# xmindflow/deformableLKA

Hardware: AMD Instinct MI355X
Metric: 3D D-LKA fwd+bwd volumes/sec (64x128x128, b2) (higher is better)
Workload: dtype f32; 1 GPU; 3D D-LKA Former Synapse 64x128x128 patch: fwd+bwd of its 21 D-LKA attention blocks (6x(32,32^3)+6x(64,16^3)+6x(128,8^3)+3x(256,4^3)) + grad all-reduce + SGD update; batch_per_gpu=2, global_batch=2, parallelism=dp1, block_params=15390693, hipgraph=True, weight_gradients_on_side_stream=True, allreduce_overlap=False, allreduce_split_block=0

## Files before the change

### deformablelka_amd/_lib.py

```python
from __future__ import annotations

import ctypes
import os
from ctypes import POINTER, c_char_p, c_int, c_int32, c_int64, c_size_t, c_void_p

import torch

_HERE = os.path.dirname(os.path.abspath(__file__))
LIB_PATH = os.path.join(_HERE, "_lib", "libdlka_hip.so")

DLKA_F32, DLKA_BF16, DLKA_F64 = 0, 1, 2
DLKA_TILES_MAX_T, DLKA_TILES_K_MAX = 64, 32
DLKA_TILES_IDENTITY, DLKA_TILES_SOFTMAX, DLKA_TILES_SIGMOID = 0, 1, 2
LKA3D_SYNAPSE, LKA3D_ACDC = 0, 1


class ConvGeom(ctypes.Structure):
    _fields_ = [(n, c_int32) for n in (
        "B", "C", "D", "H", "W", "Cout", "kd", "kh", "kw", "sd", "sh", "sw", "pd", "ph", "pw", "dd", "dh", "dw",
        "group", "deformable_group", "im2col_step")]


LKA3D_FIELDS = ("proj_1_w", "proj_1_b", "conv0_w", "conv0_b", "conv_spatial_w", "conv_spatial_b", "offset_w", "offset_b",
                "deform_w", "deform_b", "conv1_w", "conv1_b", "proj_2_w", "proj_2_b")
# ... 66 lines not shown
    "dlka_lka3d_tokens_supported": (c_int, [c_int] * 6),
    "dlka_lka3d_tokens_saved_bytes": (c_size_t, [c_int] * 6),
    "dlka_lka3d_tokens_workspace_bytes": (c_size_t, [c_int] * 6),
    "dlka_lka3d_attention_tokens_forward": (c_int, [c_void_p, POINTER(Lka3dPtrs), c_void_p, c_void_p, c_size_t, c_void_p, c_size_t]
                                            + [c_int] * 6 + [c_void_p]),
    "dlka_lka3d_attention_tokens_forward_prepared": (c_int, [c_void_p, POINTER(Lka3dPtrs), c_void_p, c_void_p, c_size_t, c_void_p, c_size_t]
                                                     + [c_int] * 6 + [c_void_p]),
    "dlka_lka3d_tokens_prepare_plan_bytes": (c_size_t, [c_int]),
    "dlka_lka3d_tokens_prepare_plan": (c_int, [c_int, POINTER(Lka3dPtrs), POINTER(c_void_p), POINTER(c_size_t), POINTER(c_int), c_int, c_void_p, c_size_t]),
    "dlka_lka3d_tokens_prepare_run": (c_int, [c_void_p, c_void_p, c_int, c_void_p]),
    "dlka_lka3d_tokens_prepare_run_range": (c_int, [c_void_p, c_void_p, c_int, c_int, c_int, c_void_p]),
    "dlka_lka3d_tokens_partials_bytes_v": (c_size_t, [c_int] * 7),
    "dlka_wgrad_finalize_plan_bytes": (c_size_t, [c_int]),
    "dlka_wgrad_finalize_plan_init": (c_int, [c_void_p, c_size_t, c_int]),
    "dlka_lka3d_attention_tokens_backward_deferred_v": (c_int, [c_void_p, POINTER(Lka3dPtrs), c_void_p, c_void_p, c_size_t, c_void_p,
                                                               POINTER(Lka3dPtrs), c_void_p, c_size_t, c_void_p, c_size_t, c_void_p, c_int,
                                                               c_int, c_int, c_int, c_int, c_int, c_int, c_int, c_void_p]),
    "dlka_lka3d_attention_tokens_backward_phase_v": (c_int, [c_void_p, POINTER(Lka3dPtrs), c_void_p, c_void_p, c_size_t, c_void_p,
                                                            POINTER(Lka3dPtrs), c_void_p, c_size_t, c_void_p, c_size_t, c_void_p, c_int, c_int,
                                                            c_int, c_int, c_int, c_int, c_int, c_int, c_int, c_void_p]),
    "dlka_wgrad_finalize_plan_seal": (c_int, [c_void_p]),
    "dlka_wgrad_finalize_run_slot": (c_int, [c_void_p, c_int, c_void_p]),
    "dlka_wgrad_finalize_run": (c_int, [c_void_p, c_void_p, c_int, c_int, c_void_p]),
    "dlka_lka3d_attention_tokens_backward": (c_int, [c_void_p, POINTER(Lka3dPtrs), c_void_p, c_void_p, c_size_t, c_void_p,
                                                     POINTER(Lka3dPtrs), c_void_p, c_size_t] + [c_int] * 6 + [c_void_p]),
    "dlka_layernorm_tokens_forward": (c_int, [c_void_p, c_int] + [c_void_p] * 6 + [c_int] * 3 + [ctypes.c_float, c_int, c_void_p]),
    "dlka_layernorm_tokens_backward": (c_int, [c_void_p] * 9 + [c_int] * 4 + [c_void_p]),
    "dlka_scale_residual_forward": (c_int, [c_void_p] * 4 + [c_int64, c_int, c_int, c_void_p]),
    "dlka_scale_residual_backward": (c_int, [c_void_p] * 5 + [c_int64, c_int, c_int, c_void_p]),
    "dlka_batchnorm_cl_forward": (c_int, [c_void_p] * 5 + [c_int] + [c_void_p] * 2 + [c_int64, c_int, ctypes.c_float, ctypes.c_float, c_int, c_void_p]),
    "dlka_batchnorm_cl_backward": (c_int, [c_void_p] * 5 + [c_int] + [c_void_p] * 5 + [c_int64, c_int, ctypes.c_float, c_int, c_void_p]),
    "dlka_channel_scale": (c_int, [c_void_p] * 3 + [c_int, c_int64, c_int, c_int, c_void_p]),
    "dlka_batchnorm_planar_forward": (c_int, [c_void_p] * 6 + [c_int, c_int, c_int64, ctypes.c_float, c_void_p]),
    "dlka_batchnorm_planar_backward": (c_int, [c_void_p] * 8 + [c_int, c_int, c_int64, c_void_p]),
    "dlka_pointwise_planar_forward": (c_int, [c_void_p] * 4 + [c_int, c_int, c_int, c_int64, c_void_p]),
    "dlka_pointwise_planar_backward": (c_int, [c_void_p] * 6 + [c_int, c_int, c_int, c_int64, c_void_p]),
    "dlka_tblock3d_supported": (c_int, [c_int] * 6),
    "dlka_tblock3d_saved_bytes": (c_size_t, [c_int] * 6),
    "dlka_tblock3d_workspace_bytes": (c_size_t, [c_int] * 6),
    "dlka_tblock3d_forward": (c_int, [c_void_p, c_int, POINTER(TBlock3dPtrs), POINTER(Lka3dPtrs), c_void_p, c_int, c_void_p, c_void_p, c_void_p, c_size_t,
                                      c_void_p, c_size_t] + [c_int] * 5 + [ctypes.c_float, ctypes.c_float, c_int, c_void_p]),
    "dlka_tblock3d_backward": (c_int, [POINTER(TBlock3dPtrs), POINTER(Lka3dPtrs), c_void_p, c_int, c_void_p, c_void_p, c_void_p, c_size_t, c_void_p,
                                       POINTER(TBlock3dPtrs), POINTER(Lka3dPtrs), c_void_p, c_size_t] + [c_int] * 6 + [c_void_p]),
    "dlka_deform_conv2d_sample_index_path": (c_int, [c_void_p] * 3 + [_G, c_int, c_int, c_void_p]),
    "dlka_deform_dwconv2d_cl_workspace": (c_size_t, [_G, c_int, c_int]),
    "dlka_deform_dwconv2d_forward_cl": (c_int, [c_void_p] * 5 + [c_size_t, _G, c_int, c_void_p]),
    "dlka_deform_dwconv2d_backward_cl": (c_int, [c_void_p] * 8 + [c_size_t, _G, c_int, c_void_p]),
    "dlka_lka3d_force_wgrad_gather": (c_int, [c_int]),
    "dlka_fork_stats": (c_int, [c_int, POINTER(ctypes.c_int64), POINTER(ctypes.c_int64)]),
    "dlka_env_refresh": (None, []),
    "dlka_dwconv_lds_launch_count": (ctypes.c_long, []),
    "dlka_conv_brick_launch_count": (ctypes.c_long, []),
    "dlka_dwpair_launch_count": (ctypes.c_long, []),
    "dlka_dwconv_2p_launch_count": (ctypes.c_long, []),
    "dlka_conv_kw_launch_count": (ctypes.c_long, []),
    "dlka_lka3d_tokens_supported_v": (c_int, [c_int] * 7),
    "dlka_lka3d_tokens_saved_bytes_v": (c_size_t, [c_int] * 7),
    "dlka_lka3d_tokens_workspace_bytes_v": (c_size_t, [c_int] * 7),
    "dlka_lka3d_attention_tokens_forward_v": (c_int, [c_void_p, POINTER(Lka3dPtrs), c_void_p, c_void_p, c_size_t, c_void_p, c_size_t]
                                              + [c_int] * 7 + [c_void_p]),
    "dlka_lka3d_attention_tokens_backward_v": (c_int, [c_void_p, POINTER(Lka3dPtrs), c_void_p, c_void_p, c_size_t, c_void_p,
                                                       POINTER(Lka3dPtrs), c_void_p, c_size_t] + [c_int] * 7 + [c_void_p]),
    "dlka_lka3d_tokens_saved_offsets_v": (c_int, [c_int] * 7 + [POINTER(c_size_t)]),
    "dlka_tblock3d_saved_offsets_v": (c_int, [c_int] * 7 + [POINTER(c_size_t)]),
    "dlka_tblock3d_saved_activations_v": (c_int, [c_int] * 7 + [POINTER(c_size_t)]),
    "dlka_tblock3d_supported_v": (c_int, [c_int] * 7),
    "dlka_tblock3d_saved_bytes_v": (c_size_t, [c_int] * 7),
    "dlka_tblock3d_workspace_bytes_v": (c_size_t, [c_int] * 7),
    "dlka_tblock3d_forward_v": (c_int, [c_void_p, c_int, POINTER(TBlock3dPtrs), POINTER(Lka3dPtrs), c_void_p, c_int, c_void_p, c_void_p, c_void_p, c_size_t,
                                        c_void_p, c_size_t] + [c_int] * 5 + [ctypes.c_float, ctypes.c_float, c_int, c_int, c_void_p]),
    "dlka_tblock3d_backward_v": (c_int, [POINTER(TBlock3dPtrs), POINTER(Lka3dPtrs), c_void_p, c_int, c_void_p, c_void_p, c_void_p, c_size_t, c_void_p,
                                         POINTER(TBlock3dPtrs), POINTER(Lka3dPtrs), c_void_p, c_size_t] + [c_int] * 7 + [c_void_p]),
    "dlka_tblock3d_backward_phase_v": (c_int, [POINTER(TBlock3dPtrs), POINTER(Lka3dPtrs), c_void_p, c_int, c_void_p, c_void_p, c_void_p, c_size_t, c_void_p,
                                         POINTER(TBlock3dPtrs), POINTER(Lka3dPtrs), c_void_p, c_size_t] + [c_int] * 8 + [c_void_p]),
    "dlka_tiles_gather": (c_int, [c_void_p] + [c_int] * 4 + [POINTER(c_int), c_int, POINTER(c_int)] + [c_int] * 7 + [ctypes.c_float, c_void_p, c_void_p]),
    "dlka_tiles_blend": (c_int, [c_void_p, c_int, c_int, c_int, ctypes.c_float] + [c_void_p] * 3 + [c_int] * 3
                         + [POINTER(c_int), c_int, POINTER(c_int)] + [c_int] * 4 + [c_void_p]),
    "dlka_tiles_finalize": (c_int, [c_void_p] * 2 + [c_int] * 10 + [c_void_p] * 3),
    "dlka_tiles_launch_count": (ctypes.c_long, []),
    "dlka_trace_start": (c_int, [c_int, c_void_p]),
    "dlka_trace_mark": (c_int, [c_void_p]),
    "dlka_trace_stop": (c_int, []),
    "dlka_trace_count": (c_int, []),
    "dlka_trace_get": (c_int, [c_int, ctypes.c_char_p, c_size_t, POINTER(ctypes.c_float)]),
}


def bind(cdll: ctypes.CDLL) -> ctypes.CDLL:
    for name, (res, args) in SIGNATURES.items():
        fn = getattr(cdll, name)
        fn.restype = res
        fn.argtypes = args
    if cdll.dlka_abi_version() != 1:
        raise RuntimeError("libdlka ABI version mismatch")
    return cdll


_lib = None
_test_backend = False


def get_lib() -> ctypes.CDLL:
    global _lib
    if _lib is None:
        if not os.path.exists(LIB_PATH):
            raise RuntimeError(
# ... 56 lines not shown
```

### deformablelka_amd/csrc/cl_host_ops.hip

```cpp
#include <atomic>
#include <mutex>

#include "cl_host.h"

namespace dlka {

int make_same_conv(const dlka_conv_geom *c, SameConv &s)
{
    if (!c) return DLKA_ERR_NULL;
    if (c->B <= 0 || c->C <= 0 || c->D <= 0 || c->H <= 0 || c->W <= 0 || c->Cout <= 0) return DLKA_ERR_SHAPE;
    if (c->kd <= 0 || c->kh <= 0 || c->kw <= 0 || c->dd <= 0 || c->dh <= 0 || c->dw <= 0) return DLKA_ERR_SHAPE;
    if (c->group <= 0 || c->C % c->group || c->Cout % c->group) return DLKA_ERR_GROUP;
    if (c->sd != 1 || c->sh != 1 || c->sw != 1) return DLKA_ERR_UNSUPPORTED;
    if (dlka_conv_out_size(c->D, c->pd, c->dd, c->kd, 1) != c->D || dlka_conv_out_size(c->H, c->ph, c->dh, c->kh, 1) != c->H ||
        dlka_conv_out_size(c->W, c->pw, c->dw, c->kw, 1) != c->W)
        return DLKA_ERR_UNSUPPORTED;
    const long N = (long)c->D * c->H * c->W;
    if (N > (1l << 30) || (long)c->B * N > (1l << 30)) return DLKA_ERR_SHAPE;
    s.B = c->B; s.D = c->D; s.H = c->H; s.W = c->W; s.N = (int)N; s.M = (int)(c->B * N);
    s.Cin = c->C; s.Cout = c->Cout; s.group = c->group;
    s.kd = c->kd; s.kh = c->kh; s.kw = c->kw; s.pd = c->pd; s.ph = c->ph; s.pw = c->pw;
    s.dd = c->dd; s.dh = c->dh; s.dw = c->dw; s.K = c->kd * c->kh * c->kw;
    s.act_bf16 = 0;
    return DLKA_OK;
// ... 293 lines not shown
}

size_t deform_scratch_floats(const SameConv &s)
{
    DeformBwdArgs a;
    fill_deform_bwd(a, s);
    return cl_deform_bwd2_scratch_floats(a);
}

static bool samp_f16(const SameConv &s)
{
    static const bool on = [] { const char *e = getenv("DLKA_SAMP_F16"); return !(e && e[0] == '0') && getenv("DLKA_EXACT_FP32") == nullptr; }();
    return on && !s.act_bf16;
}

int deform_backward(const SameConv &s, const float *x, const float *off, const float *w, const float *gout, float *gx, float *goff,
                    float *gw, float *gb, float *wp, float *part, float *scratch, hipStream_t st, FinalizeJob *defer, bool gx_zeroed,
                    bool goff_zeroed, int goff_cpad, float *samp, const float *wp16)
{
    if (gx || goff) {
        if (w) DLKA_TRY(launch_cl_prep_weight(w, wp, s.Cout, s.Cin, s.K, s.Cout, s.Cin, 2, st));
        DeformBwdArgs a;
        fill_deform_bwd(a, s);
        a.in = x; a.off = off; a.g = gout; a.wp = wp; a.gx = gx; a.goff = goff; a.gx_zeroed = gx_zeroed ? 1 : 0; a.goff_zeroed = goff_zeroed ? 1 : 0; a.goff_cpad = goff_cpad;
        a.samp = goff ? samp : nullptr;
        a.samp_f16 = (a.samp && samp_f16(s)) ? 1 : 0;
        a.wp16 = deform_b16() ? wp16 : nullptr;
        DLKA_TRY(launch_cl_deform_bwd2(a, scratch, st));
    }
    if (gw) {
        WgradArgs a;
        memset(&a, 0, sizeof(a));
        a.g = gout; a.in = x; a.off = off; a.part = part; a.samp = samp;
        a.samp_f16 = (samp && samp_f16(s)) ? 1 : 0;
        {
            static const bool b16 = [] { const char *e = getenv("DLKA_SAMP_B16MFMA"); return !(e && e[0] == '0'); }();
            a.samp_b16mfma = (a.samp_f16 && b16) ? 1 : 0;
        }
        copy_geom(a, s);
        a.Cin = s.Cin; a.Cout = s.Cout;
        a.act_bf16 = s.act_bf16;
        DLKA_TRY(launch_cl_wgrad<float>(1, 0, a, gw, gb, st, defer));
    } else if (gb) {
        if (s.act_bf16) return DLKA_ERR_UNSUPPORTED;
        DLKA_TRY(launch_cl_colsum(gout, gb, s.M, s.Cout, st));
    }
    return DLKA_OK;
}

int pointwise_pair(const SameConv &s, int bwd, const float *in, const float *wp1, const float *bias1, const float *wp2, const float *bias2,
                   const float *a, const float *b, float *out1, float *out1b, float *out2, hipStream_t st, const ZeroBatch *ride)
{
    const bool unfused = getenv("DLKA_PW_UNFUSED") != nullptr;
    if (unfused || s.Cin != 32 || s.Cin != s.Cout || s.K != 1) return DLKA_ERR_UNSUPPORTED;
    PwPairArgs pa;
    memset(&pa, 0, sizeof(pa));
    pa.in = in; pa.wp1 = wp1; pa.bias1 = bias1; pa.wp2 = wp2; pa.bias2 = bias2; pa.a = a; pa.b = b;
    pa.out1 = out1; pa.out1b = out1b; pa.out2 = out2; pa.M = s.M; pa.C = s.Cin; pa.bwd = bwd; pa.act_bf16 = s.act_bf16;
    if (ride) pa.zero = *ride;
    return launch_cl_pointwise_pair(pa, st);
}

static std::atomic<int> g_wgrad_gather{-1};
bool wgrad_gather()
{
    int v = g_wgrad_gather.load(std::memory_order_acquire);
    if (v < 0) {
        int want = getenv("DLKA_WGRAD_GATHER") != nullptr ? 1 : 0;
        if (g_wgrad_gather.compare_exchange_strong(v, want, std::memory_order_acq_rel)) v = want;
    }
    return v != 0;
}

void add_job(PrepBatch &pb, const void *src, float *dst, int Cout, int Cin, int K, int KP, int NP, int mode)
{
    PrepJob &j = pb.j[pb.njobs++];
    j.src = (const float *)src; j.dst = dst; j.Cout = Cout; j.Cin = Cin; j.K = K; j.KP = KP; j.NP = NP; j.mode = mode;
    if (!fork_env().prep_tiled && (mode & 7) <= 2) j.mode |= 32;
    j.n = (mode == 3 || mode == 4) ? (long)Cin * K : (long)K * KP * NP;
    pb.total += j.n;
}

}

using namespace dlka;

extern "C" {

void dlka_env_refresh(void)
{
    fork_env_load();
}

int dlka_lka3d_force_wgrad_gather(int on)
{
    const int old = wgrad_gather() ? 1 : 0;
    g_wgrad_gather.store(on ? 1 : 0, std::memory_order_release);
    return old;
}

}
```

### deformablelka_amd/csrc/cl_pointwise.hip

```cpp
#include "cl_args.h"
#include "dlka_kernels.h"

namespace dlka {

template <typename T, int KW = 1>
__global__ __launch_bounds__(64 * KW, 2) void cl_pointwise_kernel(IgemmArgs p)
{
    constexpr unsigned SB = sizeof(T);
    const T *auxp = reinterpret_cast<const T *>(p.aux), *aux2p = reinterpret_cast<const T *>(p.aux2);
    T *outp = reinterpret_cast<T *>(p.out), *out2p = reinterpret_cast<T *>(p.out2);
    const int lane = threadIdx.x & 63, kwave = KW > 1 ? (int)(threadIdx.x >> 6) : 0, i = lane & 31, h = lane >> 5;
    if (p.zero_xblocks && (int)blockIdx.x >= (int)gridDim.x - p.zero_xblocks) {
        if (kwave == 0) zero_batch_block(p.zero, (blockIdx.x - (gridDim.x - p.zero_xblocks)) * gridDim.y + blockIdx.y, lane, 64);
        return;
    }
    const int mbase = blockIdx.x * 32, n0 = blockIdx.y * 32;
    const int m = mbase + i, n = n0 + i;
    const BufRsrc rin = make_rsrc(p.in, (size_t)p.M * p.Cin * SB);
    const BufRsrc rw = make_rsrc(p.wp, (size_t)p.CinP * p.NP * 4);
    const unsigned abase = m < p.M ? (unsigned)m * (unsigned)p.Cin * SB + 16u * SB * h : DLKA_OOB;
    const unsigned bbase = ((unsigned)(16 * h) * (unsigned)p.NP + (unsigned)n) * 4u;
    const unsigned bstep = (unsigned)p.NP * 4u;
    f32x16 acc;
#pragma unroll
    for (int r = 0; r < 16; ++r) acc[r] = 0.f;
    float auxv[16], aux2v[16];
    const bool n_ok = n < p.Cout;
    constexpr bool B16 = sizeof(T) == 2;
    const bool odd = i & 1;
    unsigned auxw[8], aux2w[8];
    auto pair_request = [&](const T *src, int r) -> unsigned {
        const int mrow = mbase + (r & 3) + 8 * (r >> 2) + 4 * h + (odd ? 1 : 0);
        return (n_ok && mrow < p.M) ? *reinterpret_cast<const unsigned *>(src + ((long)mrow * p.Cout + (n & ~1))) : 0u;
    };
    auto pair_finish = [&](unsigned own, float &x0, float &x1) {
        const unsigned oth = lane_xor1(own);
        x0 = __uint_as_float(odd ? (oth & 0xffff0000u) : (own << 16));
        x1 = __uint_as_float(odd ? (own & 0xffff0000u) : (oth << 16));
    };
    if (p.epi >= 2 && kwave == 0) {
        if (B16) {
#pragma unroll
            for (int r = 0; r < 16; r += 2) {
                auxw[r >> 1] = pair_request(auxp, r);
                aux2w[r >> 1] = p.epi == 4 ? pair_request(aux2p, r) : 0u;
            }
        } else {
#pragma unroll
            for (int r = 0; r < 16; ++r) {
                const int mr = mbase + (r & 3) + 8 * (r >> 2) + 4 * h;
                const bool ok = n_ok && mr < p.M;
                auxv[r] = ok ? act_load1(auxp, (long)mr * p.Cout + n) : 0.f;
// ... 189 lines not shown
#pragma unroll
        for (int r = 0; r < 16; ++r) acc[r] = 0.f;
#pragma unroll
        for (int u = 0; u < NTC; ++u) {
            float b[16];
#pragma unroll
            for (int s = 0; s < 16; ++s) b[s] = buf_load_f32(rw1, (unsigned)((u * 32 + 16 * h + s) * C + n) * 4u);
#pragma unroll
            for (int s = 0; s < 16; ++s) acc = mfma_32x32x2(a[u][s >> 2][s & 3], b[s], acc);
        }
        const float bias = (!p.bwd && p.bias1) ? p.bias1[n] : 0.f;
        float t1[16], t2[16];
#pragma unroll
        for (int r = 0; r < 16; ++r) {
            const float t = acc[r] + bias;
            if (p.bwd) { t1[r] = t * av[r]; t2[r] = t * bv2[r]; }
            else { t1[r] = t; t2[r] = av[r] * t; }
        }
        store_tile(o1, nt, t1);
        store_tile(o1b, nt, t2);
#pragma unroll
        for (int r = 0; r < 16; ++r) Tm[((r & 3) + 8 * (r >> 2) + 4 * h) * LD + n] = stored(p.bwd ? t1[r] : t2[r]);
    }
    wave_sync();
    f32x4 a2[NTC][4];
#pragma unroll
    for (int u = 0; u < NTC; ++u)
#pragma unroll
        for (int e = 0; e < 4; ++e) a2[u][e] = *reinterpret_cast<const f32x4 *>(Tm + i * LD + u * 32 + 16 * h + 4 * e);
#pragma unroll 1
    for (int nt = 0; nt < NTC; ++nt) {
        const int n = nt * 32 + i;
        float res[16];
        if (!p.bwd) load_tile(bp, nt, res);
        f32x16 acc;
#pragma unroll
        for (int r = 0; r < 16; ++r) acc[r] = 0.f;
#pragma unroll
        for (int u = 0; u < NTC; ++u) {
            float b[16];
#pragma unroll
            for (int s = 0; s < 16; ++s) b[s] = buf_load_f32(rw2, (unsigned)((u * 32 + 16 * h + s) * C + n) * 4u);
#pragma unroll
            for (int s = 0; s < 16; ++s) acc = mfma_32x32x2(a2[u][s >> 2][s & 3], b[s], acc);
        }
        const float bias = (!p.bwd && p.bias2) ? p.bias2[n] : 0.f;
        float y[16];
#pragma unroll
        for (int r = 0; r < 16; ++r) y[r] = p.bwd ? acc[r] : acc[r] + bias + res[r];
        store_tile(o2, nt, y);
    }
}

int launch_cl_pointwise_pair(const PwPairArgs &a, hipStream_t st)
{
    if ((a.C != 32 && a.C != 64) || (long)a.M * a.C * 4 >= (1l << 31)) return DLKA_ERR_UNSUPPORTED;
    PwPairArgs ax = a;
    ax.zero_blocks = 0;
    unsigned blocks = (unsigned)cdiv(a.M, 32);
    if (a.zero.n > 0) {
        if (a.zero.overflow) return DLKA_ERR_WORKSPACE;
        unsigned blk = 0;
        for (int r = 0; r < a.zero.n; ++r) {
            if ((uintptr_t)a.zero.p[r] & 15) return DLKA_ERR_UNSUPPORTED;
            ax.zero.block0[r] = blk;
            blk += (unsigned)cdivl(a.zero.cnt[r], 4096);
        }
        ax.zero.block0[a.zero.n] = blk;
        ax.zero_blocks = (int)blk;
        blocks += blk;
    }
    dim3 grid(blocks), block(64);
    if (a.act_bf16) {
        if (a.C == 32) { auto k = cl_pointwise_pair_kernel<bf16_t, 1>; DLKA_LAUNCH(k, grid, block, 0, st, ax); }
        else { auto k = cl_pointwise_pair_kernel<bf16_t, 2>; DLKA_LAUNCH(k, grid, block, 0, st, ax); }
    } else {
        if (a.C == 32) { auto k = cl_pointwise_pair_kernel<float, 1>; DLKA_LAUNCH(k, grid, block, 0, st, ax); }
        else { auto k = cl_pointwise_pair_kernel<float, 2>; DLKA_LAUNCH(k, grid, block, 0, st, ax); }
    }
    DLKA_CHECK_LAUNCH();
    return DLKA_OK;
}

int launch_cl_pointwise(const IgemmArgs &a, hipStream_t st)
{
    if (a.K != 1 || a.split_bf16 || a.Cin % 32 || a.CinP != a.Cin || a.NP % 32) return DLKA_ERR_UNSUPPORTED;
    if ((long)a.M * a.Cin * 4 >= (1l << 31) || (long)a.CinP * a.NP * 4 >= (1l << 31)) return DLKA_ERR_UNSUPPORTED;
    dim3 grid(cdiv(a.M, 32), a.NP / 32), block(64);
    IgemmArgs ax = a;
    ax.zero_xblocks = 0;
    if (a.zero.n > 0) {
        if (a.zero.overflow) return DLKA_ERR_WORKSPACE;
        unsigned blk = 0;
        for (int r = 0; r < a.zero.n; ++r) {
            if ((uintptr_t)a.zero.p[r] & 15) return DLKA_ERR_UNSUPPORTED;
            ax.zero.block0[r] = blk;
            blk += (unsigned)cdivl(a.zero.cnt[r], 4096);
        }
        ax.zero.block0[a.zero.n] = blk;
        ax.zero_xblocks = (int)cdiv((int)blk, (int)grid.y);
        grid.x += ax.zero_xblocks;
    }
    const char *ekw = getenv("DLKA_PW_KW");
    const bool kw4 = ekw ? atoi(ekw) == 4 : ((long)cdiv(a.M, 32) * (a.NP / 32) <= 256 && a.CinP >= 128);
    if (kw4) {
        block = dim3(256);
        if (a.act_bf16) { auto k = cl_pointwise_kernel<bf16_t, 4>; DLKA_LAUNCH(k, grid, block, 0, st, ax); }
        else { auto k = cl_pointwise_kernel<float, 4>; DLKA_LAUNCH(k, grid, block, 0, st, ax); }
    } else if (a.act_bf16) { auto k = cl_pointwise_kernel<bf16_t>; DLKA_LAUNCH(k, grid, block, 0, st, ax); }
    else { auto k = cl_pointwise_kernel<float>; DLKA_LAUNCH(k, grid, block, 0, st, ax); }
    DLKA_CHECK_LAUNCH();
    return DLKA_OK;
}

}
```

### deformablelka_amd/csrc/dlka_kernels.h

```cpp
#pragma once
#include "cl_args.h"
#include "dlka_common.h"

namespace dlka {

int deform_pick_cob(int Og);
int deform_fwd_wt_floats(const Geom &g);
template <typename T>
int launch_relayout_weight(const T *w, float *wt, int group, int Og, int Cg, int K, int OgP, hipStream_t st);
template <typename T, int NOFF>
int launch_deform_fwd(const T *x, const T *off, const T *w, const T *bias, T *out, float *wt, const Geom &g, hipStream_t st);
template <typename T, int NOFF>
int launch_deform_bwd_input_offset(const T *x, const T *off, const float *wt, int OgP, const T *gout,
                                   float *gx32, T *goff, const Geom &g, hipStream_t st);
template <typename T, int NOFF>
int launch_deform_bwd_weight(const T *x, const T *off, const T *gout, float *gw32, const Geom &g, hipStream_t st);
template <typename T>
int launch_bias_grad(const T *gout, T *gb, int B, int Cout, int No, hipStream_t st);
template <typename T>
int launch_cast_from_f32(const float *src, T *dst, long n, hipStream_t st);
template <typename T>
int launch_sample_index(const T *off, int32_t *idx, uint8_t *mask, const Geom &g, int path, hipStream_t st);
template <typename T>
int launch_sample_index2(const T *off, int32_t *idx, uint8_t *mask, const Geom &g, int path, hipStream_t st);

template <int NOFF> int launch_deform_fwd_f64(const double *x, const double *off, const double *w, const double *bias, double *out, const Geom &g, hipStream_t st);
template <int NOFF> int launch_deform_bwd_f64(const double *x, const double *off, const double *w, const double *gout, double *gx, double *goff, double *gw, double *gb,
                                              const Geom &g, hipStream_t st);
int launch_conv_fwd_f64(const double *x, const double *w, const double *bias, double *out, const Geom &g, hipStream_t st);
int launch_conv_bwd_f64(const double *x, const double *w, const double *gout, double *gx, double *gw, double *gb, const Geom &g, hipStream_t st);

int conv_fwd_wt_floats(const Geom &g);
int conv_bwd_wb_floats(const Geom &g);
template <typename T>
int launch_conv_fwd(const T *x, const T *w, const T *bias, T *out, float *wt, const Geom &g, hipStream_t st);
template <typename T>
int launch_conv_bwd_data(const T *gout, const T *w, T *gx, float *wb, const Geom &g, hipStream_t st);
size_t conv_bwd_weight_part_floats(const Geom &g, size_t elem_bytes);
template <typename T>
int launch_conv_bwd_weight(const T *x, const T *gout, float *gw32, const Geom &g, hipStream_t st, float *part = nullptr);

int launch_zero(void *ptr, size_t bytes, hipStream_t st);
struct ZeroBatch;
int launch_zero_batch(ZeroBatch &b, hipStream_t st);
template <typename T> int launch_gelu_fwd(const T *x, T *y, long n, hipStream_t st);
template <typename T> int launch_gelu_bwd(const T *x, const T *gy, T *gx, long n, hipStream_t st);
template <typename T> int launch_mul_fwd(const T *a, const T *b, T *y, long n, hipStream_t st);
template <typename T> int launch_mul_bwd(const T *a, const T *b, const T *gy, T *ga, T *gb, long n, hipStream_t st);
template <typename T> int launch_add_fwd(const T *a, const T *b, T *y, long n, hipStream_t st);
template <typename T> int launch_gelu_bwd_sum(const T *x, const T *g1, const T *g2, T *gx, long n, hipStream_t st);

int launch_cl_prep_weight(const float *w, float *wp, int Cout, int Cin, int K, int KP, int NP, int mode, hipStream_t st);
int launch_cl_prep_batch(const PrepBatch &b, hipStream_t st);
int cl_prep_table_blocks(const PrepJob &j);
int launch_cl_prep_table(const PrepJob *jobs_dev, const int *first_dev, int job_lo, int job_hi, int nblocks, hipStream_t st);
int cl_igemm_pick_splits(int M, int units, int epi, int K);
int launch_cl_pointwise(const IgemmArgs &a, hipStream_t st);
int launch_cl_pointwise_pair(const PwPairArgs &a, hipStream_t st);
int launch_cl_conv_wave(int amode, int omode, const IgemmArgs &a, int splits, hipStream_t st);
bool cl_conv_kw_applies(int amode, int omode, int split_bf16, int K, int epi, int NP, bool act_bf16, bool volume);
int launch_cl_conv_kw(int amode, int omode, const IgemmArgs &a, hipStream_t st);
bool cl_conv_brick_supported(const IgemmArgs &a);
int cl_conv_brick_split(const IgemmArgs &a);
bool cl_conv_brick3_supported(const IgemmArgs &a);
int launch_cl_conv_brick3(const IgemmArgs &a, hipStream_t st);
int launch_cl_conv_brick(const IgemmArgs &a, hipStream_t st);
int launch_cl_igemm(int amode, int omode, IgemmArgs a, int splits, hipStream_t st);
int launch_cl_deform_fwd(IgemmArgs a, int splits, hipStream_t st);
int cl_deform_fwd_actual_splits(int K, int CinP, int splits);
int launch_cl_slab_reduce(const float *slab, int S, long n, void *out, int out_bf16, hipStream_t st);
int cl_wgrad_pick_chunks(int M, int K, int Cout, int Cin, int amode);
size_t cl_wgrad_part_floats(int M, int K, int Cout, int Cin);
size_t cl_wgrad_pad_bytes(int B, int D, int H, int W, int Cin, int kd, int kh, int kw, int dd, int dh, int dw, int act_bf16);
template <typename T> int launch_cl_wgrad(int amode, int gmode, WgradArgs a, T *gw, T *gb, hipStream_t st, FinalizeJob *defer = nullptr);
size_t cl_wgrad_part_floats_mode(int M, int K, int Cout, int Cin, int amode);
int launch_cl_wgrad_finalize(FinalizeBatch &b, hipStream_t st);
int launch_pl_bn_forward(const float *x, const float *w, const float *b, float *stats, float *y, float *scratch, int B, int C, long N, float eps, hipStream_t st);
int launch_pl_bn_backward(const float *g, const float *x, const float *w, const float *stats, float *gx, float *gw, float *gb, float *scratch, int B, int C,
                          long N, hipStream_t st);
int launch_pl_pw_forward(const float *x, const float *w, const float *bias, float *y, int B, int CI, int CO, long N, hipStream_t st);
int launch_pl_pw_backward(const float *x, const float *w, const float *g, float *gx, float *gw, float *gb, int B, int CI, int CO, long N, hipStream_t st);
long cl_wgrad_finalize_plan_job(FinalizeJob &j);
int launch_cl_wgrad_finalize_table(const FinalizeJob *jobs_device, int job_lo, int job_hi, long nblocks, hipStream_t st);
int launch_cl_wgrad_pw3(const WgradArgs *jobs, float *const *gw, float *const *gb, hipStream_t st, FinalizeJob *defer);
int launch_cl_colsum(const float *g, float *gb32, int M, int Cout, hipStream_t st);
int launch_cl_dw_prep_weight(const float *w, float *wp, int C, int K, int flip, hipStream_t st);
int launch_cl_dwconv(const DwArgs &a, int kw, int dil_w, hipStream_t st);
bool cl_dwpair_small_supported(const DwPairArgs &a);
int launch_cl_dwpair_small(const DwPairArgs &a, hipStream_t st);
int launch_cl_dwconv_lds(const DwArgs &a, int kw, int dil_w, hipStream_t st);
bool cl_dwconv_lds_selected(const DwArgs &a, int kw, int dil_w);
int cl_dwconv_lds_mode();
size_t cl_dwconv_blk_floats(int B, int C, int D, int H, int W, int dil);
int launch_cl_dwconv_wgrad(DwWgradArgs a, int kw, int dil_w, hipStream_t st, bool zero_init = true);
template <typename T> int launch_cl_dw_unprep(const float *gwp, T *gw, int C, int K, hipStream_t st);
int launch_cl_transpose(const float *src, float *dst, int B, int C, int N, int to_cl, hipStream_t st, int bf16 = 0);
size_t cl_deform_bwd2_scratch_floats(const DeformBwdArgs &a);
int launch_cl_deform_bwd2(const DeformBwdArgs &a, float *scratch, hipStream_t st);
int cl_deform_goff_ccsplit(const DeformBwdArgs &a);

int cl_ddw2d_supported(int C);
size_t cl_ddw2d_part_floats(int M, int K, int C);
int launch_cl_ddw2d_fwd(const DwArgs2d &d, hipStream_t st);
int launch_cl_ddw2d_bwd(const DwArgs2d &d, float *gw, hipStream_t st, hipStream_t gx_st = nullptr);
int lka2d_cl_supported(int B, int C, int H, int W, int dtype);
size_t lka2d_cl_saved_bytes(int B, int C, int H, int W, int dtype);
int lka2d_cl_saved_offsets(int B, int C, int H, int W, int dtype, size_t byte_offsets[2], int *elem_bytes);
size_t lka2d_cl_workspace_bytes(int B, int C, int H, int W, int dtype);
int lka2d_cl_forward(const void *x, const dlka_lka2d_params *p, void *y, void *saved, size_t saved_bytes, void *workspace, size_t workspace_bytes, int B,
                     int C, int H, int W, int dtype, hipStream_t st);
int lka2d_cl_backward(const void *x, const dlka_lka2d_params *p, const void *gy, const void *saved, size_t saved_bytes, void *gx, const dlka_lka2d_grads *gr,
// ... 17 lines not shown
```

### include/dlka.h

```cpp
#ifndef DLKA_H_
#define DLKA_H_

#include <stddef.h>
#include <stdint.h>

#ifdef __cplusplus
extern "C" {
#endif

#define DLKA_ABI_VERSION 1

typedef enum dlka_status {
    DLKA_OK = 0,
    DLKA_ERR_NULL = -1,
    DLKA_ERR_GROUP = -2,
    DLKA_ERR_DEFORM_GROUP = -3,
    DLKA_ERR_SHAPE = -4,
    DLKA_ERR_IM2COL_STEP = -5,
    DLKA_ERR_DTYPE = -6,
    DLKA_ERR_WORKSPACE = -7,
    DLKA_ERR_UNSUPPORTED = -8,
    DLKA_ERR_LAUNCH = -9
} dlka_status;

// ... 191 lines not shown
                                  int B, int C, int64_t N, float eps, void *stream);
int dlka_batchnorm_planar_backward(const void *g, const void *x, const void *w, const void *stats, void *gx, void *gw, void *gb,
                                   void *scratch, int B, int C, int64_t N, void *stream);
int dlka_pointwise_planar_forward(const void *x, const void *w, const void *bias, void *y, int B, int Cin, int Cout, int64_t N, void *stream);
int dlka_pointwise_planar_backward(const void *x, const void *w, const void *g, void *gx, void *gw, void *gb,
                                   int B, int Cin, int Cout, int64_t N, void *stream);

typedef struct dlka_tblock3d_params {
    const void *norm_w, *norm_b;
    const void *gamma;
    const void *pos_embed;
    const void *conv51_conv1_w, *conv51_conv2_w;
    const void *conv51_norm1_w, *conv51_norm1_b;
    const void *conv51_norm2_w, *conv51_norm2_b;
    const void *conv8_w, *conv8_b;
} dlka_tblock3d_params;

typedef struct dlka_tblock3d_grads {
    void *norm_w, *norm_b, *gamma, *pos_embed, *conv51_conv1_w, *conv51_conv2_w, *conv51_norm1_w, *conv51_norm1_b,
         *conv51_norm2_w, *conv51_norm2_b, *conv8_w, *conv8_b;
} dlka_tblock3d_grads;

int dlka_tblock3d_supported(int B, int C, int D, int H, int W, int dtype);
size_t dlka_tblock3d_saved_bytes(int B, int C, int D, int H, int W, int dtype);
size_t dlka_tblock3d_workspace_bytes(int B, int C, int D, int H, int W, int dtype);
int dlka_tblock3d_forward(const void *x, int x_planar, const dlka_tblock3d_params *p, const dlka_lka3d_params *lka,
                          const void *drop_mask, int training, void *bn_stats, void *y,
                          void *saved, size_t saved_bytes, void *workspace, size_t workspace_bytes,
                          int B, int C, int D, int H, int W, float ln_eps, float bn_eps, int dtype, void *stream);
int dlka_tblock3d_backward(const dlka_tblock3d_params *p, const dlka_lka3d_params *lka, const void *drop_mask, int training,
                           const void *bn_stats, const void *grad_y, const void *saved, size_t saved_bytes, void *grad_x,
                           const dlka_tblock3d_grads *grads, const dlka_lka3d_grads *lka_grads,
                           void *workspace, size_t workspace_bytes, int B, int C, int D, int H, int W, int dtype, void *stream);

int dlka_deform_conv2d_sample_index_path(const void *offset, int32_t *idx, uint8_t *mask,
                                         const dlka_conv_geom *g, int dtype, int path, void *stream);

size_t dlka_deform_dwconv2d_cl_workspace(const dlka_conv_geom *g, int dtype, int backward);
int dlka_deform_dwconv2d_forward_cl(const void *x, const void *offset, const void *weight, void *out,
                                    void *workspace, size_t workspace_bytes, const dlka_conv_geom *g, int dtype, void *stream);
int dlka_deform_dwconv2d_backward_cl(const void *x, const void *offset, const void *weight, const void *grad_out,
                                     void *grad_x, void *grad_offset, void *grad_weight,
                                     void *workspace, size_t workspace_bytes, const dlka_conv_geom *g, int dtype, void *stream);

typedef enum dlka_lka3d_variant { DLKA_LKA3D_SYNAPSE = 0, DLKA_LKA3D_ACDC = 1 } dlka_lka3d_variant;
int    dlka_lka3d_tokens_supported_v(int B, int C, int D, int H, int W, int dtype, int variant);
size_t dlka_lka3d_tokens_saved_bytes_v(int B, int C, int D, int H, int W, int dtype, int variant);
int dlka_lka3d_force_wgrad_gather(int on);
int  dlka_fork_stats(int device, int64_t *contexts, int64_t *leases);
void dlka_env_refresh(void);
long dlka_dwconv_lds_launch_count(void);
long dlka_conv_brick_launch_count(void);
long dlka_dwpair_launch_count(void);
long dlka_conv_kw_launch_count(void);
long dlka_dwconv_2p_launch_count(void);
size_t dlka_lka3d_tokens_workspace_bytes_v(int B, int C, int D, int H, int W, int dtype, int variant);
int dlka_lka3d_attention_tokens_forward_v(const void *x, const dlka_lka3d_params *p, void *y, void *saved, size_t saved_bytes,
                                          void *workspace, size_t workspace_bytes, int B, int C, int D, int H, int W, int dtype, int variant, void *stream);
int dlka_lka3d_attention_tokens_backward_v(const void *x, const dlka_lka3d_params *p, const void *grad_y, const void *saved, size_t saved_bytes,
                                           void *grad_x, const dlka_lka3d_grads *grads, void *workspace, size_t workspace_bytes,
                                           int B, int C, int D, int H, int W, int dtype, int variant, void *stream);
int    dlka_tblock3d_supported_v(int B, int C, int D, int H, int W, int dtype, int variant);
size_t dlka_tblock3d_saved_bytes_v(int B, int C, int D, int H, int W, int dtype, int variant);
int dlka_lka3d_tokens_saved_offsets_v(int B, int C, int D, int H, int W, int dtype, int variant, size_t *byte_offset);
int dlka_tblock3d_saved_offsets_v(int B, int C, int D, int H, int W, int dtype, int variant, size_t *byte_offset);
int dlka_tblock3d_saved_activations_v(int B, int C, int D, int H, int W, int dtype, int variant, size_t byte_offsets[2]);
size_t dlka_tblock3d_workspace_bytes_v(int B, int C, int D, int H, int W, int dtype, int variant);
int dlka_tblock3d_forward_v(const void *x, int x_planar, const dlka_tblock3d_params *p, const dlka_lka3d_params *lka,
                            const void *drop_mask, int training, void *bn_stats, void *y, void *saved, size_t saved_bytes,
                            void *workspace, size_t workspace_bytes, int B, int C, int D, int H, int W, float ln_eps, float bn_eps,
                            int dtype, int variant, void *stream);
int dlka_tblock3d_backward_v(const dlka_tblock3d_params *p, const dlka_lka3d_params *lka, const void *drop_mask, int training,
                             const void *bn_stats, const void *grad_y, const void *saved, size_t saved_bytes, void *grad_x,
                             const dlka_tblock3d_grads *grads, const dlka_lka3d_grads *lka_grads,
                             void *workspace, size_t workspace_bytes, int B, int C, int D, int H, int W, int dtype, int variant, void *stream);
int dlka_tblock3d_backward_phase_v(const dlka_tblock3d_params *p, const dlka_lka3d_params *lka, const void *drop_mask, int training, const void *bn_stats,
                                   const void *grad_y, const void *saved, size_t saved_bytes, void *grad_x, const dlka_tblock3d_grads *grads,
                                   const dlka_lka3d_grads *lka_grads, void *workspace, size_t workspace_bytes, int B, int C, int D, int H, int W, int dtype,
                                   int variant, int phase, void *stream);

#define DLKA_TILES_MAX_T 64
#define DLKA_TILES_K_MAX 32
#define DLKA_TILES_IDENTITY 0
#define DLKA_TILES_SOFTMAX 1
#define DLKA_TILES_SIGMOID 2
int dlka_tiles_gather(const float *x, int C, int X, int Y, int Z, const int *origins, int T, const int *masks, int M, int pd, int ph,
                      int pw, int pad_x, int pad_y, int pad_z, float pad_value, float *out, void *stream);
int dlka_tiles_blend(const void *logits, int dtype, int K, int nonlin, float mirror_scale, const float *gauss, float *score,
                     float *weight, int Xp, int Yp, int Zp, const int *origins, int T, const int *masks, int M, int pd, int ph, int pw,
                     void *stream);
int dlka_tiles_finalize(const float *score, const float *weight, int K, int Xp, int Yp, int Zp, int pad_x, int pad_y, int pad_z, int X,
                        int Y, int Z, float *probs, int64_t *seg, void *stream);
long dlka_tiles_launch_count(void);

int dlka_trace_start(int max_events, void *stream);
int dlka_trace_mark(void *stream);
int dlka_trace_stop(void);
int dlka_trace_count(void);
int dlka_trace_get(int i, char *name, size_t name_cap, float *ms);

#ifdef __cplusplus
}
#endif
#endif
```

Measured before the change: 208.5 volumes/s.

## Add fused pointwise-chain kernel for 64/128/256-channel 1x1 conv pairs

Extends the fused pointwise pair (two chained 1x1 convs with gating and residual, forward and backward) beyond 32 channels. A new MFMA kernel handles C=64 directly and C=128/256 by splitting the contraction across waves with an LDS reduction. The intermediate tile stays in shared memory instead of taking a round trip through global memory and a second launch. C=128 only runs when the grid is small, and C=256 needs an env flag. The old C=64 path inside the pair kernel is dropped in favour of the new kernel, and the extra LDS and larger blocks may reduce occupancy.

```diff
diff --git a/deformablelka_amd/_lib.py b/deformablelka_amd/_lib.py
--- a/deformablelka_amd/_lib.py
+++ b/deformablelka_amd/_lib.py
@@ -142,6 +142,7 @@
     "dlka_dwconv_lds_launch_count": (ctypes.c_long, []),
     "dlka_conv_brick_launch_count": (ctypes.c_long, []),
     "dlka_dwpair_launch_count": (ctypes.c_long, []),
+    "dlka_pw_chain_launch_count": (ctypes.c_long, []),
     "dlka_dwconv_2p_launch_count": (ctypes.c_long, []),
     "dlka_conv_kw_launch_count": (ctypes.c_long, []),
     "dlka_lka3d_tokens_supported_v": (c_int, [c_int] * 7),
diff --git a/deformablelka_amd/csrc/cl_host_ops.hip b/deformablelka_amd/csrc/cl_host_ops.hip
--- a/deformablelka_amd/csrc/cl_host_ops.hip
+++ b/deformablelka_amd/csrc/cl_host_ops.hip
@@ -369,13 +369,13 @@
                    const float *a, const float *b, float *out1, float *out1b, float *out2, hipStream_t st, const ZeroBatch *ride)
 {
     const bool unfused = getenv("DLKA_PW_UNFUSED") != nullptr;
-    if (unfused || s.Cin != 32 || s.Cin != s.Cout || s.K != 1) return DLKA_ERR_UNSUPPORTED;
+    if (unfused || s.Cin != s.Cout || s.K != 1) return DLKA_ERR_UNSUPPORTED;
     PwPairArgs pa;
     memset(&pa, 0, sizeof(pa));
     pa.in = in; pa.wp1 = wp1; pa.bias1 = bias1; pa.wp2 = wp2; pa.bias2 = bias2; pa.a = a; pa.b = b;
     pa.out1 = out1; pa.out1b = out1b; pa.out2 = out2; pa.M = s.M; pa.C = s.Cin; pa.bwd = bwd; pa.act_bf16 = s.act_bf16;
     if (ride) pa.zero = *ride;
-    return launch_cl_pointwise_pair(pa, st);
+    return s.Cin == 32 ? launch_cl_pointwise_pair(pa, st) : launch_cl_pointwise_chain(pa, st);
 }
 
 static std::atomic<int> g_wgrad_gather{-1};
diff --git a/deformablelka_amd/csrc/cl_pointwise.hip b/deformablelka_amd/csrc/cl_pointwise.hip
--- a/deformablelka_amd/csrc/cl_pointwise.hip
+++ b/deformablelka_amd/csrc/cl_pointwise.hip
@@ -1,3 +1,5 @@
+#include <atomic>
+
 #include "cl_args.h"
 #include "dlka_kernels.h"
 
@@ -293,33 +295,228 @@
     }
 }
 
+static int pair_zero_blocks(const PwPairArgs &a, PwPairArgs &ax, unsigned &blocks)
+{
+    ax.zero_blocks = 0;
+    if (a.zero.n <= 0) return DLKA_OK;
+    if (a.zero.overflow) return DLKA_ERR_WORKSPACE;
+    unsigned blk = 0;
+    for (int r = 0; r < a.zero.n; ++r) {
+        if ((uintptr_t)a.zero.p[r] & 15) return DLKA_ERR_UNSUPPORTED;
+        ax.zero.block0[r] = blk;
+        blk += (unsigned)cdivl(a.zero.cnt[r], 4096);
+    }
+    ax.zero.block0[a.zero.n] = blk;
+    ax.zero_blocks = (int)blk;
+    blocks += blk;
+    return DLKA_OK;
+}
+
 int launch_cl_pointwise_pair(const PwPairArgs &a, hipStream_t st)
 {
-    if ((a.C != 32 && a.C != 64) || (long)a.M * a.C * 4 >= (1l << 31)) return DLKA_ERR_UNSUPPORTED;
+    if (a.C != 32 || (long)a.M * a.C * 4 >= (1l << 31)) return DLKA_ERR_UNSUPPORTED;
     PwPairArgs ax = a;
-    ax.zero_blocks = 0;
     unsigned blocks = (unsigned)cdiv(a.M, 32);
-    if (a.zero.n > 0) {
-        if (a.zero.overflow) return DLKA_ERR_WORKSPACE;
-        unsigned blk = 0;
-        for (int r = 0; r < a.zero.n; ++r) {
-            if ((uintptr_t)a.zero.p[r] & 15) return DLKA_ERR_UNSUPPORTED;
-            ax.zero.block0[r] = blk;
-            blk += (unsigned)cdivl(a.zero.cnt[r], 4096);
-        }
-        ax.zero.block0[a.zero.n] = blk;
-        ax.zero_blocks = (int)blk;
-        blocks += blk;
-    }
+    if (const int rc = pair_zero_blocks(a, ax, blocks)) return rc;
     dim3 grid(blocks), block(64);
+    if (a.act_bf16) { auto k = cl_pointwise_pair_kernel<bf16_t, 1>; DLKA_LAUNCH(k, grid, block, 0, st, ax); }
+    else { auto k = cl_pointwise_pair_kernel<float, 1>; DLKA_LAUNCH(k, grid, block, 0, st, ax); }
+    DLKA_CHECK_LAUNCH();
+    return DLKA_OK;
+}
+
+template <typename T, int NTC, int KW, int KWW>
+__global__ __launch_bounds__(64 * NTC * KWW) void cl_pointwise_chain_kernel(PwPairArgs p)
+{
+    constexpr unsigned SB = sizeof(T);
+    constexpr bool B16 = SB == 2;
+    constexpr int C = NTC * 32, LD = C + 4, KS = KW / KWW, NCH = NTC / KW;
+    constexpr int NRED = KW - KS;
+    static_assert(KW % KWW == 0 && NTC % KW == 0 && NCH <= 4, "slice split");
+    __shared__ __attribute__((aligned(16))) float Tm[32 * LD];
+    __shared__ __attribute__((aligned(16))) float red[(NRED > 0 ? NRED * NTC : 1) * 16 * 64];
+    const int tid = threadIdx.x, lane = tid & 63, wave = tid >> 6, kwave = wave % KWW, ct = wave / KWW, i = lane & 31, h = lane >> 5;
+    const int mtiles = (int)gridDim.x - p.zero_blocks;
+    if ((int)blockIdx.x >= mtiles) {
+        zero_batch_block(p.zero, blockIdx.x - mtiles, tid, 64 * NTC * KWW);
+        return;
+    }
+    const T *ap = reinterpret_cast<const T *>(p.a), *bp = reinterpret_cast<const T *>(p.b);
+    T *o1 = reinterpret_cast<T *>(p.out1), *o1b = reinterpret_cast<T *>(p.out1b), *o2 = reinterpret_cast<T *>(p.out2);
+    const int mbase = blockIdx.x * 32, m = mbase + i, n = ct * 32 + i;
+    const bool odd = i & 1, lead = kwave == 0;
+    const BufRsrc rin = make_rsrc(p.in, (size_t)p.M * C * SB);
+    const BufRsrc rw1 = make_rsrc(p.wp1, (size_t)C * C * 4), rw2 = make_rsrc(p.wp2, (size_t)C * C * 4);
+    const unsigned abase = m < p.M ? (unsigned)m * (unsigned)C * SB + 16u * SB * h : DLKA_OOB;
+    auto row_of = [&](int r) { return mbase + (r & 3) + 8 * (r >> 2) + 4 * h; };
+    auto tile_request = [&](const T *src, unsigned *w) {
+        if (B16) {
+#pragma unroll
+            for (int r = 0; r < 16; r += 2) {
+                const int mrow = row_of(r) + (odd ? 1 : 0);
+                w[r >> 1] = mrow < p.M ? *reinterpret_cast<const unsigned *>(src + ((long)mrow * C + (n & ~1))) : 0u;
+            }
+        } else {
+#pragma unroll
+            for (int r = 0; r < 16; ++r) w[r] = row_of(r) < p.M ? __float_as_uint(act_load1(src, (long)row_of(r) * C + n)) : 0u;
+        }
+    };
+    auto tile_finish = [&](const unsigned *w, float *v) {
+        if (B16) {
+#pragma unroll
+            for (int r = 0; r < 16; r += 2) {
+                const unsigned own = w[r >> 1], oth = lane_xor1(own);
+                v[r] = __uint_as_float(odd ? (oth & 0xffff0000u) : (own << 16));
+                v[r + 1] = __uint_as_float(odd ? (own & 0xffff0000u) : (oth << 16));
+            }
+        } else {
+#pragma unroll
+            for (int r = 0; r < 16; ++r) v[r] = __uint_as_float(w[r]);
+        }
+    };
+    auto store_tile = [&](T *dst, const float *v) {
+        if (B16) {
+#pragma unroll
+            for (int r = 0; r < 16; r += 2) {
+                const unsigned give = bf16_bits(odd ? v[r] : v[r + 1]), mine = bf16_bits(odd ? v[r + 1] : v[r]);
+                const unsigned got = lane_xor1(give);
+                const unsigned word = odd ? (got | (mine << 16)) : (mine | (got << 16));
+                const int mrow = row_of(r) + (odd ? 1 : 0);
+                if (mrow < p.M) *reinterpret_cast<unsigned *>(dst + ((long)mrow * C + (n & ~1))) = word;
+            }
+        } else {
+#pragma unroll
+            for (int r = 0; r < 16; ++r)
+                if (row_of(r) < p.M) act_store1(dst, (long)row_of(r) * C + n, v[r]);
+        }
+    };
+    auto stored = [&](float x) { return B16 ? bf16_value(bf16_bits(x)) : x; };
+    auto contract = [&](bool second, BufRsrc rw, f32x16 *acc) {
+#pragma unroll
+        for (int j = 0; j < KS; ++j) {
+            const int ks = kwave + KWW * j;
+#pragma unroll
+            for (int r = 0; r < 16; ++r) acc[j][r] = 0.f;
+            f32x4 a[NCH][4];
+            float b[NCH][16];
+#pragma unroll
+            for (int u = 0; u < NCH; ++u) {
+                const int ck = ks + u * KW;
+                if (second) {
+#pragma unroll
+                    for (int e = 0; e < 4; ++e) a[u][e] = *reinterpret_cast<const f32x4 *>(Tm + i * LD + ck * 32 + 16 * h + 4 * e);
+                } else {
+                    const unsigned ao = abase == DLKA_OOB ? DLKA_OOB : abase + (unsigned)ck * 32u * SB;
+                    if (B16) {
+                        buf_load_bf16x8(rin, ao, a[u][0], a[u][1]);
+                        buf_load_bf16x8(rin, ao == DLKA_OOB ? DLKA_OOB : ao + 16u, a[u][2], a[u][3]);
+                    } else {
+#pragma unroll
+                        for (int e = 0; e < 4; ++e) a[u][e] = act_buf_load4<T>(rin, ao == DLKA_OOB ? DLKA_OOB : ao + 16u * e);
+                    }
+                }
+#pragma unroll
+                for (int s = 0; s < 16; ++s) b[u][s] = buf_load_f32(rw, (unsigned)((ck * 32 + 16 * h + s) * C + n) * 4u);
+            }
+#pragma unroll
+            for (int u = 0; u < NCH; ++u)
+#pragma unroll
+                for (int s = 0; s < 16; ++s) acc[j] = mfma_32x32x2(a[u][s >> 2][s & 3], b[u][s], acc[j]);
+            if (KS > 1) sched_fence();
+        }
+    };
+    auto fold = [&](f32x16 *acc) {
+        if (KW == 1) return;
+        if (!lead) {
+#pragma unroll
+            for (int j = 0; j < KS; ++j) {
+                const int ks = kwave + KWW * j, slot = ct * NRED + ks - 1 - ks / KWW;
+#pragma unroll
+                for (int r = 0; r < 16; r += 4)
+                    *reinterpret_cast<f32x4 *>(&red[(slot * 16 + r) * 64 + 4 * lane]) = f32x4{acc[j][r], acc[j][r + 1], acc[j][r + 2], acc[j][r + 3]};
+            }
+        }
+        __syncthreads();
+        if (!lead) return;
+#pragma unroll
+        for (int ks = 1; ks < KW; ++ks) {
+            if (ks % KWW == 0) {
+#pragma unroll
+                for (int r = 0; r < 16; ++r) acc[0][r] += acc[ks / KWW][r];
+            } else {
+                const int slot = ct * NRED + ks - 1 - ks / KWW;
+#pragma unroll
+                for (int r = 0; r < 16; r += 4) {
+                    const f32x4 o = *reinterpret_cast<const f32x4 *>(&red[(slot * 16 + r) * 64 + 4 * lane]);
+                    acc[0][r] += o[0]; acc[0][r + 1] += o[1]; acc[0][r + 2] += o[2]; acc[0][r + 3] += o[3];
+                }
+            }
+        }
+    };
+
+    unsigned aw[16], bw[16];
+    if (lead) {
+        tile_request(ap, aw);
+        if (p.bwd) tile_request(bp, bw);
+    }
+    f32x16 acc[KS];
+    contract(false, rw1, acc);
+    fold(acc);
+    if (lead) {
+        float av[16], bv2[16], t1[16], t2[16];
+        tile_finish(aw, av);
+        if (p.bwd) tile_finish(bw, bv2);
+        const float bias = (!p.bwd && p.bias1) ? p.bias1[n] : 0.f;
+#pragma unroll
+        for (int r = 0; r < 16; ++r) {
+            const float t = acc[0][r] + bias;
+            if (p.bwd) { t1[r] = t * av[r]; t2[r] = t * bv2[r]; }
+            else { t1[r] = t; t2[r] = av[r] * t; }
+        }
+        store_tile(o1, t1);
+        store_tile(o1b, t2);
+#pragma unroll
+        for (int r = 0; r < 16; ++r) Tm[((r & 3) + 8 * (r >> 2) + 4 * h) * LD + n] = stored(p.bwd ? t1[r] : t2[r]);
+        if (!p.bwd) tile_request(bp, bw);
+    }
+    __syncthreads();
+    contract(true, rw2, acc);
+    fold(acc);
+    if (lead) {
+        float res[16], y[16];
+        if (!p.bwd) tile_finish(bw, res);
+        const float bias = (!p.bwd && p.bias2) ? p.bias2[n] : 0.f;
+#pragma unroll
+        for (int r = 0; r < 16; ++r) y[r] = p.bwd ? acc[0][r] : acc[0][r] + bias + res[r];
+        store_tile(o2, y);
+    }
+}
+
+static std::atomic<long> g_pw_chain_launches{0};
+
+int launch_cl_pointwise_chain(const PwPairArgs &a, hipStream_t st)
+{
+    if ((a.C != 64 && a.C != 128 && a.C != 256) || (long)a.M * a.C * 4 >= (1l << 31)) return DLKA_ERR_UNSUPPORTED;
+    if (getenv("DLKA_PW_KW")) return DLKA_ERR_UNSUPPORTED;
+    if (a.C >= 128 && (long)cdiv(a.M, 32) * (a.C / 32) > 256) return DLKA_ERR_UNSUPPORTED;
+    if (a.C == 256 && !getenv("DLKA_PW_CHAIN_256")) return DLKA_ERR_UNSUPPORTED;
+    PwPairArgs ax = a;
+    unsigned blocks = (unsigned)cdiv(a.M, 32);
+    if (const int rc = pair_zero_blocks(a, ax, blocks)) return rc;
+    dim3 grid(blocks);
+#define DLKA_CHAIN(T, NTC, KW, KWW) do { auto k = cl_pointwise_chain_kernel<T, NTC, KW, KWW>; DLKA_LAUNCH(k, grid, dim3(64 * NTC * KWW), 0, st, ax); } while (0)
     if (a.act_bf16) {
-        if (a.C == 32) { auto k = cl_pointwise_pair_kernel<bf16_t, 1>; DLKA_LAUNCH(k, grid, block, 0, st, ax); }
-        else { auto k = cl_pointwise_pair_kernel<bf16_t, 2>; DLKA_LAUNCH(k, grid, block, 0, st, ax); }
+        if (a.C == 64) DLKA_CHAIN(bf16_t, 2, 1, 1);
+        else if (a.C == 128) DLKA_CHAIN(bf16_t, 4, 4, 4);
+        else DLKA_CHAIN(bf16_t, 8, 4, 2);
     } else {
-        if (a.C == 32) { auto k = cl_pointwise_pair_kernel<float, 1>; DLKA_LAUNCH(k, grid, block, 0, st, ax); }
-        else { auto k = cl_pointwise_pair_kernel<float, 2>; DLKA_LAUNCH(k, grid, block, 0, st, ax); }
-    }
+        if (a.C == 64) DLKA_CHAIN(float, 2, 1, 1);
+        else if (a.C == 128) DLKA_CHAIN(float, 4, 4, 4);
+        else DLKA_CHAIN(float, 8, 4, 2);
+    }
+#undef DLKA_CHAIN
     DLKA_CHECK_LAUNCH();
+    g_pw_chain_launches.fetch_add(1, std::memory_order_relaxed);
     return DLKA_OK;
 }
 
@@ -355,3 +552,5 @@
 }
 
 }
+
+extern "C" long dlka_pw_chain_launch_count(void) { return dlka::g_pw_chain_launches.load(std::memory_order_relaxed); }
diff --git a/deformablelka_amd/csrc/dlka_kernels.h b/deformablelka_amd/csrc/dlka_kernels.h
--- a/deformablelka_amd/csrc/dlka_kernels.h
+++ b/deformablelka_amd/csrc/dlka_kernels.h
@@ -57,6 +57,7 @@
 int cl_igemm_pick_splits(int M, int units, int epi, int K);
 int launch_cl_pointwise(const IgemmArgs &a, hipStream_t st);
 int launch_cl_pointwise_pair(const PwPairArgs &a, hipStream_t st);
+int launch_cl_pointwise_chain(const PwPairArgs &a, hipStream_t st);
 int launch_cl_conv_wave(int amode, int omode, const IgemmArgs &a, int splits, hipStream_t st);
 bool cl_conv_kw_applies(int amode, int omode, int split_bf16, int K, int epi, int NP, bool act_bf16, bool volume);
 int launch_cl_conv_kw(int amode, int omode, const IgemmArgs &a, hipStream_t st);
diff --git a/include/dlka.h b/include/dlka.h
--- a/include/dlka.h
+++ b/include/dlka.h
@@ -267,6 +267,7 @@
 long dlka_dwconv_lds_launch_count(void);
 long dlka_conv_brick_launch_count(void);
 long dlka_dwpair_launch_count(void);
+long dlka_pw_chain_launch_count(void);
 long dlka_conv_kw_launch_count(void);
 long dlka_dwconv_2p_launch_count(void);
 size_t dlka_lka3d_tokens_workspace_bytes_v(int B, int C, int D, int H, int W, int dtype, int variant);
```

Measured after the change: 211.5 volumes/s (median of 6 runs). 1.01x the previous value.
